# slimgroup/SetIntersectionProjection.jl

Hardware: AMD Instinct MI355X
Metric: PARSDMM iterations/sec (higher is better)
Workload: dtype f32

## Files before the change

setintersectionprojection.jl_amd/csrc/engine.cpp:

```cpp
#include "engine.h"
#include "comm.h"
#include "device_memory.h"
#include "dist_dft.h"
#include "ext_proj.h"
#include "host_prefault.h"
#include "set_config.h"
#include "solve_rules.h"
#include "sparse_granules.h"

#include <algorithm>
#include <array>
#include <chrono>
#include <cmath>
#include <cstdio>
#include <cstdlib>
#include <cstring>
#include <limits>
#include <thread>
#include <exception>

namespace sipx {

const LaunchObserver*& launch_observer() {
  static thread_local const LaunchObserver* obs = nullptr;
// ... 3043 lines not shown
    std::vector<KAgg> agg = aggregate_samples();
    const KAgg& a = stencil_q_ ? agg[KID_SQ_DOT] : agg[KID_CDS_DOT];
    if (launches) *launches = a.launches;
    if (total_ms) *total_ms = a.ms;
    start_stats(enable);
  }
  const char* kernel_stats_json(int enable) override {
    const bool peek = enable < 0;
    if (!peek) need_final();
    std::vector<KAgg> agg = peek ? std::vector<KAgg>(KID_COUNT) : aggregate_samples();
    std::string& o = stats_json_;
    o = "{\"mode\": " + std::to_string(stats_mode_) + ", \"event_pair_overhead_ms\": " + std::to_string(stat_pair_ms_) + ", \"kernels\": [";
    bool first = true;
    char buf[512];
    for (int k = 0; k < KID_COUNT; ++k) {
      if (!agg[k].launches) continue;
      const bool gated = gated_kernel(k);
      std::snprintf(buf, sizeof buf,
                    "%s{\"name\": \"%s\", \"launches\": %lld, \"noop_launches\": %lld, \"total_ms\": %.6f, \"bytes_survey\": %.0f, "
                    "\"bytes_moved\": %.0f, \"gated\": %s, \"inclusive\": %s}",
                    first ? "" : ", ", kernel_name(k), (long long)agg[k].launches, (long long)agg[k].noops, agg[k].ms, agg[k].bytes_survey,
                    agg[k].bytes_moved,
                    gated ? "true" : "false", k == KID_EXT ? "true" : "false");
      o += buf;
      first = false;
    }
    o += "], \"slab_searches\": {\"speculative_exchange\": " + std::to_string(spec_searches_) + ", \"fallbacks\": " +
         std::to_string(spec_fallbacks_) + ", \"refinement_rounds\": " + std::to_string(spec_rounds_) + "}";
    o += std::string(", \"sparse_arrays\": ") + (slab_local_ ? "true" : "false");
    {
      std::string loc, fan;
      for (int i = 0; i < p_n_; ++i) {
        if (sets_[i].slab_ext || sets_[i].slab_card || sets_[i].slab_dft) loc += (loc.empty() ? "" : ", ") + std::to_string(i);
        if (sets_[i].fan) fan += (fan.empty() ? "" : ", ") + std::to_string(i);
      }
      if (counting_)
        o += ", \"collectives\": {\"allreduce\": " + std::to_string(counting_->n_allreduce) + ", \"allreduce_with_halo\": " + std::to_string(counting_->n_grouped) +
             ", \"allgather\": " + std::to_string(counting_->n_allgather) + ", \"reduce_scatter\": " + std::to_string(counting_->n_reduce_scatter) +
             ", \"halo\": " + std::to_string(counting_->n_halo) + ", \"scatter_gather\": " + std::to_string(counting_->n_fan) +
             ", \"alltoall\": " + std::to_string(counting_->n_alltoall) + "}";
      o += ", \"slab_loose\": {\"slab_local_sets\": [" + loc + "], \"gathered_sets\": [" + fan + "], \"fan_exchanges\": " + std::to_string(fan_exchanges_) + "}";
    }
    {
      std::string t = selftest_;
      for (auto& ch : t) if (ch == '"' || ch == '\\' || (unsigned char)ch < 32) ch = ' ';
      o += ", \"comm_selftest\": \"" + t + "\"";
    }
    o += ", \"lane_set\": " + std::to_string(lane_set_);
    o += std::string(", \"q_table\": {\"on\": ") + (cds_.qtab ? "true" : "false") + ", \"reason\": \"" + qtab_reason_ + "\"}";
    o += ", \"batched_searches\": {\"searches\": " + std::to_string(batch_searches_) + ", \"fallbacks\": " + std::to_string(batch_fallbacks_) + "}";
    o += ", \"routes\": {";
    for (int r = 0; r < RT_COUNT; ++r) o += std::string(r ? ", \"" : "\"") + route_name(r) + "\": " + std::to_string(routes_[r]);
    o += "}";
    long long rc[4] = {project_rc_[0], project_rc_[1], project_rc_[2], project_rc_[3]};
    for (const auto& st : sets_) {
      if (!st.ext || st.ext_kind != EXT_RANK) continue;
      long long c[4];
      st.ext->route_counts(c);
      for (int q = 0; q < 4; ++q) rc[q] += c[q];
    }
    o += ", \"rank_route\": {\"calls\": " + std::to_string(rc[0]) + ", \"warm_started_subspace\": " + std::to_string(rc[1]) +
         ", \"full_decomposition\": " + std::to_string(rc[2]) + ", \"products_with_gram\": " + std::to_string(rc[3]) + "}";
    long long fc[4] = {0, 0, 0, 0};
    for (const auto& st : sets_) {
      if (!st.ext || st.ext_kind != EXT_L21_SEG) continue;
      long long c[4];
      st.ext->route_counts(c);
      fc[0] += c[0]; fc[1] = std::max(fc[1], c[1]); fc[3] += c[3];
    }
    o += ", \"l21_frames\": {\"passes_total\": " + std::to_string(fc[0]) + ", \"passes_max\": " + std::to_string(fc[1]) +
         ", \"frames\": " + std::to_string(fc[3]) + "}";
    long long wc[4] = {0, 0, 0, 0};
    for (const auto& st : sets_) {
      if (!st.ext || !st.weighted) continue;
      long long c[4];
      st.ext->route_counts(c);
      for (int q = 0; q < 4; ++q) wc[q] += c[q];
    }
    o += ", \"l21_weighted\": {\"passes\": " + std::to_string(wc[0]) + ", \"flag_reads\": " + std::to_string(wc[1]) +
         ", \"calls\": " + std::to_string(wc[2]) + ", \"groups\": " + std::to_string(wc[3]) + "}}";
    if (!peek) start_stats(enable);
    return o.c_str();
  }
  double stat_pair_overhead_ms() const { return stat_pair_ms_; }

  void debug_proj(int set, int which, double* o) override {
    need_final();
    for (int k = 0; k < 16; ++k) o[k] = 0;
    if (set < 0 || set >= p_n_) throw std::runtime_error("set index out of range");
    const ProjScalars<T>* d = (which & 1) ? sets_[set].psf : sets_[set].ps;
    if (!d) return;
    ProjScalars<T> h;
    SIPX_HIP(hipStreamSynchronize(stream_));
    SIPX_HIP(hipMemcpy(&h, d, sizeof(h), hipMemcpyDeviceToHost));
    o[0] = h.need; o[1] = h.theta; o[2] = h.theta_prev; o[3] = h.hw; o[4] = h.spec_lo; o[5] = h.spec_hi; o[6] = h.lo;
    o[7] = h.hi; o[8] = h.asum; o[9] = h.vmax; o[10] = h.dbg[0]; o[11] = h.dbg[1]; o[12] = h.dbg[2]; o[13] = h.dbg[3];
    o[14] = h.refine;
    o[15] = h.lean + 2 * h.dbg_sampled;
    if (which & 2) { o[4] = h.samp_theta; o[5] = h.samp_lo; o[6] = h.samp_hi; o[7] = h.samp_c; }
  }

  void* stream() override { return (void*)stream_; }
  void* dev_rhs() override { return rhs_; }
  void* dev_x() override { return x_; }
  void get_rhs(void* out) override {
    need_final();
    if (slab_local_ && comm_->world > 1) throw std::runtime_error("a slab-decomposed context holds its planes of rhs only");
    SIPX_HIP(hipStreamSynchronize(stream_));
    SIPX_HIP(hipMemcpy(out, rhs_, Nx_ * sizeof(T), hipMemcpyDeviceToHost));
  }

 private:
  struct KSample { int kid; double bytes_survey, bytes_moved; };
  struct KAgg { long long launches = 0, noops = 0; double ms = 0, bytes_survey = 0, bytes_moved = 0; };
  hipEvent_t stat_event(size_t i) {
    while (stat_ev_.size() <= i) {
      hipEvent_t e;
      SIPX_HIP(hipEventCreate(&e));
      stat_ev_.push_back(e);
    }
    return stat_ev_[i];
  }
  static void obs_begin(void* user, int kid, hipStream_t s, double bytes_survey, double bytes_moved) {
    auto* e = static_cast<Engine<T>*>(user);
    if (e->stats_mode_ == 0 || (e->stats_mode_ == 1 && kid != KID_CDS_DOT && kid != KID_SQ_DOT)) return;
    const size_t i = e->samples_.size();
    e->samples_.push_back(KSample{kid, bytes_survey, bytes_moved});
    e->open_.push_back(i);
    SIPX_HIP(hipEventRecord(e->stat_event(2 * i), s));
  }
  static void obs_end(void* user, int kid, hipStream_t s) {
    auto* e = static_cast<Engine<T>*>(user);
    if (e->stats_mode_ == 0 || (e->stats_mode_ == 1 && kid != KID_CDS_DOT && kid != KID_SQ_DOT)) return;
    if (e->open_.empty()) return;
    const size_t i = e->open_.back();
    e->open_.pop_back();
    if (i < e->samples_.size()) SIPX_HIP(hipEventRecord(e->stat_event(2 * i + 1), s));
  }
  static void obs_route(void* user, int route) {
    if (route >= 0 && route < RT_COUNT) static_cast<Engine<T>*>(user)->routes_[route] += 1;
  }
  void drop_samples_from(size_t n) {
    if (n < samples_.size()) samples_.resize(n);
    open_.clear();
  }
  void sync_all_streams() {
    SIPX_HIP(hipStreamSynchronize(stream_));
    for (hipStream_t q : pool_) if (q != stream_) SIPX_HIP(hipStreamSynchronize(q));
    if (cstream_) SIPX_HIP(hipStreamSynchronize(cstream_));
  }
  static bool gated_kernel(int k) {
    return k == KID_PASS_FIRST || k == KID_PASS_LEAN || k == KID_PASS_PROBE || k == KID_PASS_COMPACT || k == KID_SAMPLE ||
           k == KID_DECIDE || k == KID_CDS_FUSED || k == KID_CG_XR || k == KID_CG_P || k == KID_SLOT_SUMS;
  }
  std::vector<KAgg> aggregate_samples() {
    sync_all_streams();
    std::vector<KAgg> agg(KID_COUNT);
    for (size_t i = 0; i < samples_.size(); ++i) {
      float ms = 0;
      if (hipEventElapsedTime(&ms, stat_ev_[2 * i], stat_ev_[2 * i + 1]) != hipSuccess) { (void)hipGetLastError(); continue; }
      KAgg& a = agg[samples_[i].kid];
      const double t = (double)ms - stat_pair_ms_;
      a.launches += 1;
      a.ms += t > 0 ? t : 0;
      const bool noop = gated_kernel(samples_[i].kid) && samples_[i].bytes_moved > 0 && t * 1e-3 < samples_[i].bytes_moved / 16e12;
      a.noops += noop ? 1 : 0;
      a.bytes_survey += noop ? 0.0 : samples_[i].bytes_survey;
      a.bytes_moved += noop ? 0.0 : samples_[i].bytes_moved;
    }
    return agg;
  }
  void start_stats(int mode) {
    samples_.clear();
    open_.clear();
    stats_mode_ = 0;
    if (mode) {
      std::vector<float> gap;
      for (int k = 0; k < 16; ++k) {
        SIPX_HIP(hipEventRecord(stat_event(2 * k), stream_));
        SIPX_HIP(hipEventRecord(stat_event(2 * k + 1), stream_));
      }
      SIPX_HIP(hipStreamSynchronize(stream_));
      for (int k = 0; k < 16; ++k) {
        float ms = 0;
        SIPX_HIP(hipEventElapsedTime(&ms, stat_ev_[2 * k], stat_ev_[2 * k + 1]));
        gap.push_back(ms);
      }
      std::sort(gap.begin(), gap.end());
      stat_pair_ms_ = gap[gap.size() / 2];
    }
    stats_mode_ = mode;
  }
  const LaunchObserver* observer() const { return &obs_; }
// ... 506 lines not shown
  std::vector<SetState<T>> sets_;
  std::vector<int32_t> owned_;
  bool finalized_ = false, feasibility_only_ = false, any_ncvx_ = false;
  int p_n_ = 0, pp_n_ = 0;
  std::vector<T> rho_, gamma_;
  std::vector<double> feas_init_;
  T *p_base_ = nullptr, *m_base_ = nullptr, *r_base_ = nullptr, *p2_base_ = nullptr, *p2_ = nullptr;
  bool cg_fused_ = false;
  int n_mfree_ = 0;
  long long halo_ = 0;
  T *x_ = nullptr, *xold_ = nullptr, *rhs_ = nullptr, *m_ = nullptr, *r_ = nullptr, *p_ = nullptr, *Ap_ = nullptr;
  T *Q_ = nullptr, *scr_v_ = nullptr, *scr_c_ = nullptr, *maxpart_ = nullptr;
  long long* scr_i_ = nullptr;
  long long scr_c_len_ = 0;
  T* scr_w_ = nullptr;
  T *loose_v_ = nullptr, *loose_w_ = nullptr;
  bool loose_whole_ = false;
  bool need_idx_ = false, need_ext_ = false;
  CdsArgs cds_;
  bool set_streams_ = true;
  hipEvent_t ev_fork_ = nullptr, ev_fork2_ = nullptr;
  std::vector<hipStream_t> pool_;
  bool search_streams_ = false;
  int search_next_ = 0;
  int n_set_streams_ = 2, pool_next_ = 0;
  bool mk_ = false;
  long long Nx_ = 0;
  T *w_base_ = nullptr, *w_ = nullptr;
  StencilQ<T> sq_{};
  bool stencil_q_ = false;
  double *part_cg_ = nullptr, *part_tmp_ = nullptr, *part_sets_ = nullptr;
  CgState<T>*cg_dev_ = nullptr, *cg_host_ = nullptr;
  double* hres_ = nullptr;
  volatile unsigned long long* sums_word_ = nullptr;
  unsigned* sums_ticket_ = nullptr;
  unsigned long long sums_seq_ = 0;
  volatile int* hlean_ = nullptr;
  volatile int* hovf_ = nullptr;
  volatile unsigned* hverd_ = nullptr;
  unsigned spec_seq_ = 0;
  long long spec_searches_ = 0, spec_fallbacks_ = 0, spec_rounds_ = 0;
  int lane_set_ = -1;
  hipStream_t lane_st_ = nullptr;
  hipEvent_t lane_fork_ = nullptr, lane_ev_ = nullptr;
  T* lane_v_ = nullptr;
  std::thread lane_thr_;
  std::exception_ptr lane_err_;
  long long lane_sample_ = -1;
  SetArgs<T> lane_args_;
  bool sweep_partial_ = false, has_loose_ = false;
  bool sweep_plain_ = false;
  bool search_batch_ = false;
  long long batch_searches_ = 0, batch_fallbacks_ = 0;
  long long routes_[RT_COUNT] = {};
  long long project_rc_[4] = {0, 0, 0, 0};
  T* fbuf_ = nullptr;
  bool yl_multi_ = true;
  bool x0_mode_ = false;
  T *xr_base_[3] = {nullptr, nullptr, nullptr}, *xr_[3] = {nullptr, nullptr, nullptr};
  int x_cur_ = 0, x_snap_ = -1;
  bool rhs_fused_ = false;
  hipEvent_t sums_event_ = nullptr;
  std::unique_ptr<Comm> comm_;
  CountingComm* counting_ = nullptr;
  long long plane_ = 0, chunk_ = 0, r0_ = 0, r1_ = 0, qr0_ = 0, qr1_ = 0;
  int prev_ = -1, next_ = -1;
  hipStream_t cstream_ = nullptr;
  hipEvent_t ev_c_[2] = {nullptr, nullptr};
  bool rs_pending_ = false;
  double* dres_ = nullptr;
  hipEvent_t ev_sums_ = nullptr, ev_cgb_ = nullptr;
  bool sums_pending_ = false;
  T* qtab_ = nullptr;
  bool q_stale_ = false;
  std::string qtab_reason_ = "not built";
  DeviceMemory mem_;
  bool slab_dist_logs_ = false;
  bool lean_multi_ = false;
  bool head_done_ = false;
  int merged_nslots_ = 0;
  int sums_flags_ = 0;
  volatile unsigned long long* ticket_ = nullptr;
  unsigned cg_seq_ = 0;
  bool slab_req_ = false, slab_ = false;
  hipStream_t fan_st_ = nullptr;
  hipEvent_t fan_fork_ = nullptr;
  double* fan_ptmp_ = nullptr;
  T *fan_mpart_ = nullptr, *fan_c_ = nullptr;
  long long fan_exchanges_ = 0;
  bool slab_loose_ = false;
  bool slab_full_req_ = false, slab_local_ = false;
  std::string selftest_ = "none", mapped_why_;
  double* agree_buf_ = nullptr;
  bool selftest_mapped_failed_ = false, selftest_alltoall_failed_ = false;
  std::string a2a_why_;
  long long wlo_ = 0, whi_ = 0;
  Grid Gr_, Gyl_;
  ChainHooks hooks_;
  T* gbuf_ = nullptr;
  double *stage_ = nullptr, *sstage_ = nullptr;
  const ChainHooks* hooks() const { return slab_ ? &hooks_ : nullptr; }
  double obj_ss_ = 0, evo_ss_ = 0, xx_ss_ = 0;
  bool have_log_sums_ = false;
  hipEvent_t cg_ev_[2] = {nullptr, nullptr};
  std::vector<hipEvent_t> stat_ev_;
  std::vector<KSample> samples_;
  std::vector<size_t> open_;
// ... 115 lines not shown
```

setintersectionprojection.jl_amd/csrc/kernels_cds.hip:

```cpp
#include <cstdlib>
#include <stdexcept>
#include <string>

#include "sipx_device.h"
#define SIPX_CG_GRID launch_blocks(3)
#ifndef SIPX_F64_VEC
#define SIPX_F64_VEC 2
#endif

namespace sipx {

template <typename T, int V>
struct LoadStored {
  const T* __restrict__ x;
  __device__ __forceinline__ Vec<T, V> operator()(long long c) const { return ldv_u<T, V>(x + c); }
};
template <typename T, int V>
struct LoadFused {
  const T* __restrict__ r;
  const T* __restrict__ p;
  T beta;
  __device__ __forceinline__ Vec<T, V> operator()(long long c) const {
    const Vec<T, V> rv = ldv_u<T, V>(r + c), pv = ldv_u<T, V>(p + c);
    Vec<T, V> o;
#pragma unroll
    for (int k = 0; k < V; ++k) o.v[k] = rv.v[k] + beta * pv.v[k];
    return o;
  }
};

template <typename T, int V, int D, typename XL>
__device__ __forceinline__ void cds_rows(long long N, const T* __restrict__ R, const CdsArgs& a, const XL& xl, long long r,
                                         T (&acc)[V]) {
  const int d = D ? D : a.d;
#pragma unroll
  for (int k = 0; k < V; ++k) acc[k] = T(0);
  if constexpr (D > 0) {
    Vec<T, V> rv[D], xv[D];
#pragma unroll
    for (int b = 0; b < D; ++b) {
      if (a.sym) {
        rv[b] = a.off[b] >= 0 ? ldv<T, V>(R + (long long)b * N + r)
                              : ldv_u<T, V>(R + (long long)a.partner[b] * N + r + a.off[b]);
      } else {
        rv[b] = ldv_nt<T, V>(R + (long long)b * N + r);
      }
      xv[b] = xl(r + a.off[b]);
    }
#pragma unroll
    for (int b = 0; b < D; ++b) {
      const long long c = r + a.off[b];
#pragma unroll
      for (int k = 0; k < V; ++k) {
        const T t = acc[k] + rv[b].v[k] * xv[b].v[k];
        acc[k] = (c + k >= 0 && c + k < N) ? t : acc[k];
      }
// ... 260 lines not shown
        for (int k = 0; k < V; ++k) {
          const T rv[7] = {r0.v[k], k == 0 ? rl : r1.v[k - 1], r1.v[k], ru.v[k], r2.v[k], rzm.v[k], r3.v[k]};
          const T xv[7] = {x0.v[k], k == 0 ? xl : x0.v[k - 1], k == V - 1 ? xr : x0.v[k + 1], xu.v[k], xd.v[k], xm.v[k], xp.v[k]};
          const bool in[7] = {true, k > 0 || !first, k < V - 1 || !last, up, down, below, above};
          T acc = T(0);
#pragma unroll
          for (int q = 0; q < 7; ++q) {
            const int role = march_role(ORD, q);
            const T t = acc + rv[role] * xv[role];
            acc = in[role] ? t : acc;
          }
          o4.v[k] = acc;
        }
        if (MODE == 0) {
          stv_nt<T, V>(y + r, o4);
        } else if (MODE == 1 || MODE == 3) {
#pragma unroll
          for (int k = 0; k < V; ++k) acc0 += (double)x0.v[k] * (double)o4.v[k];
          stv_nt<T, V>(y + r, o4);
          if (MODE == 3) stv<T, V>(pout + r, x0);
        } else {
          Vec<T, V> o;
#pragma unroll
          for (int k = 0; k < V; ++k) {
            o.v[k] = bv.v[k] - o4.v[k];
            acc0 += (double)o.v[k] * (double)o.v[k];
            acc1 += (double)bv.v[k] * (double)bv.v[k];
          }
          stv<T, V>(y + r, o);
          if (pout) stv<T, V>(pout + r, o);
          if (xold) stv<T, V>(xold + r, x0);
        }
      }
      xm = x0; x0 = xp; rzm = r3;
    }
  }
  if (MODE != 0) {
    __shared__ double sm[2][MARCH_NT / 64];
    const double v0 = wave_sum(acc0), v1 = wave_sum(acc1);
    __syncthreads();
    if ((tid & 63) == 0) { sm[0][tid >> 6] = v0; sm[1][tid >> 6] = v1; }
    __syncthreads();
    if (tid < (MODE == 2 ? 2 : 1)) {
      double s = 0;
#pragma unroll
      for (int i = 0; i < MARCH_NT / 64; ++i) s += sm[tid][i];
      double* row = partials + (long long)tid * NB;
      row[blockIdx.x] = s;
      for (int jj = blockIdx.x + gridDim.x; jj < NB; jj += gridDim.x) row[jj] = 0.0;
    }
  }
}

struct MarchGeom {
  int lg, tiles_x, tiles_y, zchunk, grid;
  long long items;
};
template <typename T>
static bool march_geom(long long N, long long r0, long long r1, const CdsArgs& a, MarchGeom& m) {
  const int sw = env_knobs().cds_march;
  const long long zc_env = env_knobs().cds_march_zchunk;
  if (sw == 0 || !a.march || !a.sym || a.d != 7) return false;
  constexpr int V = sizeof(T) == 8 ? 2 : 4;
  const long long n1 = a.gn[0], n2 = a.gn[1], n3 = a.gn[2], st2 = n1 * n2;
  if (n1 % V != 0 || n1 * n2 * n3 != N || r0 % st2 != 0 || r1 % st2 != 0 || r1 <= r0) return false;
  const long long nvx = n1 / V;
  int lg = 0;
  while ((1 << lg) < nvx && lg < 6) ++lg;
  const int LX = 1 << lg, TY = MARCH_NT / LX;
  const int tiles_x = (int)((nvx + LX - 1) / LX), tiles_y = (int)((n2 + TY - 1) / TY);
  const long long tiles = (long long)tiles_x * tiles_y, planes = (r1 - r0) / st2;
  long long zchunk = planes * tiles / 2048;
  if (zchunk < 16) zchunk = 16;
  if (sw == 2 && zc_env > 0) zchunk = zc_env;
  if (zchunk > planes) zchunk = planes;
  const long long nchunks = (planes + zchunk - 1) / zchunk, items = tiles * nchunks;
  if (items < 384 && sw != 2) return false;
  m = MarchGeom{lg, tiles_x, tiles_y, (int)zchunk, (int)(items < NB ? items : NB), items};
  return true;
}
template <typename T>
bool K<T>::march_applies(long long N, const CdsArgs& a) {
  MarchGeom m;
  return march_geom<T>(N, 0, N, a, m);
}

template <typename T, int MODE>
static bool try_march(hipStream_t s, long long N, long long r0, long long r1, const T* R, const CdsArgs& a, const T* x, T* y, const T* b,
                      T* pout, T* xold, double* partials, const int* done, CgState<T>* st = nullptr, CgState<T>* host = nullptr,
                      unsigned long long* ticket = nullptr) {
  MarchGeom m;
  if (!march_geom<T>(N, r0, r1, a, m)) return false;
  constexpr int V = sizeof(T) == 8 ? 2 : 4;
  const long long n1 = a.gn[0], n2 = a.gn[1], n3 = a.gn[2], st2 = n1 * n2;
  const T *R0 = R + (long long)a.mb[0] * N, *R1 = R + (long long)a.mb[1] * N, *R2 = R + (long long)a.mb[2] * N, *R3 = R + (long long)a.mb[3] * N;
#define SIPX_MARCH(ORD, XT, XV)                                                                                                      \
  hipLaunchKernelGGL((k_cds_march<T, V, ORD, MODE, XT>), dim3(m.grid), dim3(MARCH_NT), 0, s, n1, n2, n3, r0 / st2, r1 / st2, R0, R1, R2, R3, x, y, b, \
                     pout, xold, partials, done, m.lg, m.tiles_x, m.tiles_y, m.zchunk, m.items, st, host, ticket, XV)
  if (a.qtab) {
    const QTab<T> tab{(const T*)a.qtab};
    if (a.march == 1) SIPX_MARCH(1, QTab<T>, tab);
    else SIPX_MARCH(2, QTab<T>, tab);
  } else if (a.march == 1) {
    SIPX_MARCH(1, NoExtra, NoExtra{});
  } else {
    SIPX_MARCH(2, NoExtra, NoExtra{});
  }
#undef SIPX_MARCH
  return true;
}

template <typename T, int MODE>
static void launch_cds(hipStream_t s, long long N, long long r0, long long r1, const T* R, const CdsArgs& a, const T* x, T* y,
                       const T* b, T* pout, T* xold, double* partials, const int* done) {
  if (a.d < 1 || a.d > MAXD) throw std::runtime_error("cds: band count out of range");
  if (r0 < 0 || r1 > N || r0 > r1) throw std::runtime_error("cds: row range outside the matrix");
  int read_bands = a.d;
  if (a.sym) { read_bands = 0; for (int b = 0; b < a.d; ++b) read_bands += a.off[b] >= 0 ? 1 : 0; }
  if (a.qtab) read_bands = 0;
  const double rw = (double)(r1 - r0) * sizeof(T), extra = MODE == 2 ? 4.0 : 2.0;
  const double moved_extra = (MODE == 2 && !xold) ? 3.0 : extra;
  ObsScope obs(MODE == 0 ? KID_CDS_SPMV : (MODE == 1 ? KID_CDS_DOT : KID_CDS_RESID), s, (a.d + extra) * rw, (read_bands + moved_extra) * rw);
  if (try_march<T, MODE>(s, N, r0, r1, R, a, x, y, b, pout, xold, partials, done)) {
    obs.route((a.qtab ? RT_CDS_MARCH_TABLE : RT_CDS_MARCH_BANDS) + MODE);
    SIPX_HIP(hipGetLastError());
    return;
  }
  if (a.qtab) throw std::runtime_error("internal: Q's class table is in use but the z-marching product does not apply");
  obs.route(RT_CDS_FLAT + MODE);
#define SIPX_CDS(V, D) \
  hipLaunchKernelGGL((k_cds<T, V, D, MODE>), dim3(fit_grid((r1 - r0) / V, SIPX_CG_GRID)), dim3(BLOCK), 0, s, N, r0, r1, R, a, x, y, b, pout, xold, partials, done)
  constexpr int VW = sizeof(T) == 8 ? SIPX_F64_VEC : 4;
  if (N % 4 == 0 && r0 % 4 == 0 && r1 % 4 == 0) {
    switch (a.d) {
      case 1: SIPX_CDS(VW, 1); break;
      case 3: SIPX_CDS(VW, 3); break;
      case 5: SIPX_CDS(VW, 5); break;
      case 7: SIPX_CDS(VW, 7); break;
      default: SIPX_CDS(VW, 0); break;
    }
  } else {
    SIPX_CDS(1, 0);
  }
#undef SIPX_CDS
  SIPX_HIP(hipGetLastError());
}

template <typename T>
void K<T>::spmv(hipStream_t s, const Grid&, long long N, const T* R, const CdsArgs& a, const T* x, T* y) {
  launch_cds<T, 0>(s, N, 0, N, R, a, x, y, nullptr, nullptr, nullptr, nullptr, nullptr);
}
template <typename T>
void K<T>::spmv_dot(hipStream_t s, long long N, long long r0, long long r1, const T* R, const CdsArgs& a, const T* p, T* Ap,
                    double* partials, const CgState<T>* st) {
  launch_cds<T, 1>(s, N, r0, r1, R, a, p, Ap, nullptr, nullptr, nullptr, partials, &st->done);
}
template <typename T>
void K<T>::resid(hipStream_t s, long long N, long long r0, long long r1, const T* R, const CdsArgs& a, const T* x, const T* b,
                 T* r, T* p, T* xold, double* partials) {
  launch_cds<T, 2>(s, N, r0, r1, R, a, x, r, b, p, xold, partials, nullptr);
}

template <typename T, int V>
__device__ __forceinline__ void stencil_rows(const Grid& G, const StencilQ<T>& q, const T* __restrict__ x, long long g,
                                             const Vec<T, V>& xc, T (&acc)[V]) {
  const Coord c = coords(G, g);
#pragma unroll
  for (int k = 0; k < V; ++k) acc[k] = q.w0 * xc.v[k];
#pragma unroll
  for (int dir = 0; dir < 3; ++dir) {
    if (!(q.mask & (1 << dir))) continue;
    const long long st = G.st[dir];
    const int nd = (int)G.n[dir], cd = coord_of(c, dir);
    const Vec<T, V> xm = ldv_u<T, V>(x + g - st), xp = ldv_u<T, V>(x + g + st);
#pragma unroll
    for (int k = 0; k < V; ++k) {
      const int ck = cd + (dir == 0 ? k : 0);
// ... 623 lines not shown
template <typename T, int V, int D>
__global__ __launch_bounds__(BLOCK) void k_cds_fused(long long N, const T* __restrict__ R, CdsArgs a, const T* __restrict__ r,
                                                     const T* __restrict__ p_old, T* __restrict__ p_new, T* __restrict__ Ap,
                                                     double* __restrict__ partials, CgState<T>* __restrict__ st,
                                                     CgState<T>* __restrict__ host, unsigned long long* ticket) {
  if (st->done) return;
  const double ss = block_sum_partials(partials + NB);
  const T rr = (T)ss;
  const T res = (T)sqrt(ss) / st->nr0;
  const bool conv = res <= st->tol;
  const T beta = rr / st->gamma;
  if (blockIdx.x == 0 && threadIdx.x == 0) {
    st->ss = ss;
    st->res_last = res;
    if (conv) {
      st->flag = 0;
      st->done = 1;
    } else {
      st->beta = beta;
    }
    st->rr = rr;
    *host = *st;
    publish_ticket(ticket, st->seq, st->iters, conv ? 1 : 0);
  }
  if (conv) return;
  const LoadFused<T, V> xl{r, p_old, beta};
  const long long nvec = N / V;
  double acc0 = 0;
  for (long long vi = (long long)blockIdx.x * BLOCK + threadIdx.x; vi < nvec; vi += (long long)gridDim.x * BLOCK) {
    const long long row = vi * V;
    T s[V];
    cds_rows<T, V, D>(N, R, a, xl, row, s);
    const Vec<T, V> pv = xl(row);
    Vec<T, V> o;
#pragma unroll
    for (int k = 0; k < V; ++k) {
      o.v[k] = s[k];
      acc0 += (double)pv.v[k] * (double)s[k];
    }
    stv<T, V>(p_new + row, pv);
    stv_nt<T, V>(Ap + row, o);
  }
  double acc[1] = {acc0};
  block_reduce_store<1>(acc, partials, 0);
}
template <typename T>
void K<T>::spmv_fused(hipStream_t s, long long N, const T* R, const CdsArgs& a, const T* r, const T* p_old, T* p_new, T* Ap,
                      double* partials, CgState<T>* st, CgState<T>* host, unsigned long long* ticket) {
  if (a.d < 1 || a.d > MAXD) throw std::runtime_error("cds: band count out of range");
  int read_bands = a.d;
  if (a.sym) { read_bands = 0; for (int b = 0; b < a.d; ++b) read_bands += a.off[b] >= 0 ? 1 : 0; }
  if (a.qtab) read_bands = 0;
  ObsScope obs(KID_CDS_FUSED, s, (a.d + 4.0) * (double)N * sizeof(T), (read_bands + 4.0) * (double)N * sizeof(T));
  if (try_march<T, 3>(s, N, 0, N, R, a, r, Ap, p_old, p_new, nullptr, partials, nullptr, st, host, ticket)) {
    obs.route((a.qtab ? RT_CDS_MARCH_TABLE : RT_CDS_MARCH_BANDS) + 3);
    SIPX_HIP(hipGetLastError());
    return;
  }
  if (a.qtab) throw std::runtime_error("internal: Q's class table is in use but the z-marching product does not apply");
  obs.route(RT_CDS_FUSED_FLAT);
#define SIPX_CDSF(V, D) \
  hipLaunchKernelGGL((k_cds_fused<T, V, D>), dim3(fit_grid(N / V, SIPX_CG_GRID)), dim3(BLOCK), 0, s, N, R, a, r, p_old, p_new, Ap, partials, st, host, ticket)
  constexpr int VW = sizeof(T) == 8 ? SIPX_F64_VEC : 4;
  if (N % 4 == 0) {
    switch (a.d) {
      case 1: SIPX_CDSF(VW, 1); break;
      case 3: SIPX_CDSF(VW, 3); break;
      case 5: SIPX_CDSF(VW, 5); break;
      case 7: SIPX_CDSF(VW, 7); break;
      default: SIPX_CDSF(VW, 0); break;
    }
  } else {
    SIPX_CDSF(1, 0);
  }
#undef SIPX_CDSF
  SIPX_HIP(hipGetLastError());
}

__global__ __launch_bounds__(BLOCK) void k_fin_sum(const double* __restrict__ partials, double* __restrict__ out_dev,
                                                   double* __restrict__ out_host, unsigned* __restrict__ ticket,
                                                   unsigned long long* __restrict__ word, unsigned long long seq) {
  const double s = block_sum_partials(partials + (long long)blockIdx.x * NB);
  if (threadIdx.x == 0) {
    if (out_dev) out_dev[blockIdx.x] = s;
    if (out_host) out_host[blockIdx.x] = s;
    if (word) {
      __threadfence_system();
      const unsigned t = __hip_atomic_fetch_add(ticket, 1u, __ATOMIC_ACQ_REL, __HIP_MEMORY_SCOPE_AGENT);
      if (t == gridDim.x - 1) {
        __hip_atomic_store(ticket, 0u, __ATOMIC_RELAXED, __HIP_MEMORY_SCOPE_AGENT);
        __threadfence_system();
        __hip_atomic_store(word, seq, __ATOMIC_RELEASE, __HIP_MEMORY_SCOPE_SYSTEM);
      }
    }
  }
}
template <typename T>
void K<T>::fin_sum(hipStream_t s, const double* partials, int nslots, double* out_dev, double* out_host, unsigned* ticket,
                   unsigned long long* word, unsigned long long seq) {
  ObsScope obs(KID_FIN_SUM, s, (double)nslots * NB * sizeof(double));
  hipLaunchKernelGGL(k_fin_sum, dim3(nslots), dim3(BLOCK), 0, s, partials, out_dev, out_host, ticket, word, seq);
  SIPX_HIP(hipGetLastError());
}

__global__ __launch_bounds__(BLOCK) void k_copy_f64(const double* __restrict__ src, double* __restrict__ dst, int n) {
  for (int i = threadIdx.x; i < n; i += BLOCK) dst[i] = src[i];
}
template <typename T>
// ... 38 lines not shown
```

setintersectionprojection.jl_amd/csrc/sipx_common.h:

```cpp
#pragma once
#include <hip/hip_runtime.h>
#include <stdint.h>
#include <cstdio>

#include "env_knobs.h"

namespace sipx {

constexpr int BLOCK = 256;
constexpr int NB = 2048;
constexpr int NB_7 = 1792;
inline int fit_grid(long long nvec, int cap) {
  const long long need = (nvec + BLOCK - 1) / BLOCK;
  return (int)(need < 1 ? 1 : (need < cap ? need : cap));
}
template <typename... P>
inline bool aligned16(const P*... p) {
  return (((reinterpret_cast<uintptr_t>(p) & 15u) == 0) && ...);
}
inline int launch_blocks(int per_cu) {
  static const int cus = [] {
    int dev = 0, n = 0;
    if (hipGetDevice(&dev) != hipSuccess || hipDeviceGetAttribute(&n, hipDeviceAttributeMultiprocessorCount, dev) != hipSuccess || n <= 0)
      n = 256;
    return n;
  }();
  const int g = per_cu * cus;
  return g < 256 ? 256 : (g > NB_7 ? NB_7 : g);
}
constexpr int MAXD = 32;
constexpr int MAX_SETS = 16;
constexpr int QT_N = 4 * 27;
constexpr int YL_SLOTS = 13;
constexpr int L1_K = 8;
#define SIPX_SOLVE_SLOTS 64
#define SIPX_MAX_WORLD 64
constexpr int GATHER_HDR = 8;
constexpr int PREP_SLOTS = 3 + 2 * L1_K;
template <typename T>
constexpr int fast_hdr() { return ((PREP_SLOTS + 4) * 8 / (int)sizeof(T) + 3) / 4 * 4; }
constexpr int SAMPLE_BINS = 1024;
constexpr int SAMPLE_MBITS = 7;

enum KernelId {
  KID_CDS_SPMV = 0, KID_CDS_DOT, KID_CDS_RESID, KID_CDS_FUSED, KID_SQ_SPMV, KID_SQ_DOT, KID_SQ_RESID, KID_CG_BEGIN, KID_CG_XR, KID_CG_P,
  KID_Q_UPDATE, KID_FIN_SUM, KID_RHS, KID_YL, KID_YL_MULTI, KID_ADJ_NORM, KID_LOG3, KID_PASS_FIRST, KID_PASS_LEAN, KID_PASS_PROBE,
  KID_PASS_COMPACT, KID_PASS_DIST, KID_PASS_STORE, KID_PASS_MULTI, KID_SLOT_SUMS, KID_DECIDE, KID_SAMPLE, KID_L1_SOLVE, KID_GATHER,
  KID_PS_RESCALE, KID_CARD, KID_EXT, KID_BB_RULE, KID_OTHER, KID_MF_FWD, KID_MF_ADJ, KID_L21_NORMS, KID_L21_FRAMES, KID_L21_SCALE,
  KID_L21J_NORMS, KID_L21J_FINISH, KID_L21J_SCALE, KID_L21W_PASS, KID_L21W_SCALE, KID_COUNT
};
inline const char* kernel_name(int k) {
  static const char* const names[KID_COUNT] = {
      "k_cds<MODE=0>", "k_cds<MODE=1>", "k_cds<MODE=2>", "k_cds_fused", "k_sq<MODE=0>", "k_sq<MODE=1>", "k_sq<MODE=2>", "k_cg_begin",
      "k_cg_update_xr", "k_cg_update_p", "k_q_update", "k_fin_sum", "k_rhs", "k_yl", "k_yl_multi", "k_adj_norm", "k_log3",
      "k_pass<M_FIRST>", "k_pass<M_LEAN>", "k_pass<M_PROBE>", "k_pass<M_COMPACT>", "k_pass<M_DIST>", "k_pass<M_STORE>", "k_pass_multi",
      "k_slot_sums", "k_decide", "k_sample", "k_l1_solve", "k_gather_pack/unpack", "k_ps_rescale", "k_card_*", "ext_proj (library-backed)",
      "k_bb_rule", "other", "k_mf_fwd", "k_mf_adj", "k_l21_norms", "k_l21_frames", "k_l21_scale",
      "k_l21j_norms", "k_l21j_finish", "k_l21j_scale", "k_l21w_part", "k_l21w_scale"};
  return (k >= 0 && k < KID_COUNT) ? names[k] : "?";
}
enum RouteId {
  RT_CDS_MARCH_BANDS = 0,
  RT_CDS_MARCH_TABLE = 4,
  RT_CDS_FLAT = 8,
  RT_CDS_FUSED_FLAT = 11,
  RT_RHS_MARCH = 12,
  RT_RHS_FLAT = 13,
  RT_COUNT = 14
};
inline const char* route_name(int r) {
  static const char* const names[RT_COUNT] = {
      "k_cds_march<MODE=0>/bands", "k_cds_march<MODE=1>/bands", "k_cds_march<MODE=2>/bands", "k_cds_march<MODE=3>/bands",
      "k_cds_march<MODE=0>/table", "k_cds_march<MODE=1>/table", "k_cds_march<MODE=2>/table", "k_cds_march<MODE=3>/table",
      "k_cds<MODE=0>", "k_cds<MODE=1>", "k_cds<MODE=2>", "k_cds_fused", "k_rhs_march", "k_rhs"};
  return (r >= 0 && r < RT_COUNT) ? names[r] : "?";
}
struct LaunchObserver {
  void* user;
  void (*begin)(void* user, int kid, hipStream_t s, double bytes_survey, double bytes_moved);
  void (*end)(void* user, int kid, hipStream_t s);
  void (*route)(void* user, int route);
};
const LaunchObserver*& launch_observer();

struct ObsScope {
  const LaunchObserver* o;
  int kid;
  hipStream_t s;
  ObsScope(int kid_, hipStream_t s_, double bytes_survey, double bytes_moved = -1.0) : o(launch_observer()), kid(kid_), s(s_) {
    if (env_knobs().trace_kernels) fprintf(stderr, "[sipx trace] %s\n", kernel_name(kid));
    if (o) o->begin(o->user, kid, s, bytes_survey, bytes_moved < 0 ? bytes_survey : bytes_moved);
  }
  ~ObsScope() {
    if (o) o->end(o->user, kid, s);
    if (env_knobs().trace_kernels) {
      (void)hipStreamSynchronize(s);
      fprintf(stderr, "[sipx trace]   done\n");
    }
  }
  void route(int r) const { if (o && o->route) o->route(o->user, r); }
  ObsScope(const ObsScope&) = delete;
  ObsScope& operator=(const ObsScope&) = delete;
};

enum { SL_RPRI = 0, SL_DY = 1, SL_HL = 2, SL_HH = 3, SL_LH = 4, SL_DL = 5, SL_GG = 6, SL_GL = 7,
       SL_FE = 8, SL_SS = 9, SL_OBJ = 10, SL_EVO = 11, SL_XX = 12,
       SL_ADJ = 13 , SL_FE2 = 14, SL_SS2 = 15  };
constexpr int SET_SLOTS = 16;

enum { F_FEAS = 1, F_BB = 2, F_FIRST = 4, F_NOSPEC = 8 ,
       F_STORE_DY = 16  };

enum { PX_BOUNDS = 0, PX_BOUNDS_VEC = 1, PX_L1 = 2, PX_L2 = 3, PX_ANNULUS = 4, PX_CARD = 5, PX_PROX_L1 = 6,
       PX_EXT = 8,
       PX_DIST = 100 };

struct Grid {
  long long n[3];
  long long N;
  long long st[3];
  unsigned m1 = 0, s1 = 0, m2 = 0, s2 = 0;
// ... 433 lines not shown
```

Before: 866.6.

## Add LDS ring-buffered z-marching CDS kernel using async global-to-LDS loads

Adds a variant of the z-marching 7-point stencil SpMV that streams planes into a multi-slot LDS ring buffer with global_load_lds, fetching several planes ahead. Waits use explicit vmcnt counts so loads overlap compute instead of holding neighbour planes in registers. A heuristic picks it for f32 with the class table when there are enough work items, and route counters record which load path ran. It relies on hand-computed outstanding-load counts and inline asm, so miscounted waits could cause races, and the larger LDS footprint limits occupancy to two workgroups per CU.

```diff
diff --git a/setintersectionprojection.jl_amd/csrc/engine.cpp b/setintersectionprojection.jl_amd/csrc/engine.cpp
--- a/setintersectionprojection.jl_amd/csrc/engine.cpp
+++ b/setintersectionprojection.jl_amd/csrc/engine.cpp
@@ -3119,6 +3119,7 @@
     o += ", \"routes\": {";
     for (int r = 0; r < RT_COUNT; ++r) o += std::string(r ? ", \"" : "\"") + route_name(r) + "\": " + std::to_string(routes_[r]);
     o += "}";
+    o += ", \"march_loads\": {\"ring\": " + std::to_string(routes_[RT_LOADS_RING]) + ", \"registers\": " + std::to_string(routes_[RT_LOADS_REGISTERS]) + "}";
     long long rc[4] = {project_rc_[0], project_rc_[1], project_rc_[2], project_rc_[3]};
     for (const auto& st : sets_) {
       if (!st.ext || st.ext_kind != EXT_RANK) continue;
@@ -3205,7 +3206,7 @@
     if (i < e->samples_.size()) SIPX_HIP(hipEventRecord(e->stat_event(2 * i + 1), s));
   }
   static void obs_route(void* user, int route) {
-    if (route >= 0 && route < RT_COUNT) static_cast<Engine<T>*>(user)->routes_[route] += 1;
+    if (route >= 0 && route < RT_ALL) static_cast<Engine<T>*>(user)->routes_[route] += 1;
   }
   void drop_samples_from(size_t n) {
     if (n < samples_.size()) samples_.resize(n);
@@ -3818,7 +3819,7 @@
   bool sweep_plain_ = false;
   bool search_batch_ = false;
   long long batch_searches_ = 0, batch_fallbacks_ = 0;
-  long long routes_[RT_COUNT] = {};
+  long long routes_[RT_ALL] = {};
   long long project_rc_[4] = {0, 0, 0, 0};
   T* fbuf_ = nullptr;
   bool yl_multi_ = true;
diff --git a/setintersectionprojection.jl_amd/csrc/kernels_cds.hip b/setintersectionprojection.jl_amd/csrc/kernels_cds.hip
--- a/setintersectionprojection.jl_amd/csrc/kernels_cds.hip
+++ b/setintersectionprojection.jl_amd/csrc/kernels_cds.hip
@@ -2,6 +2,7 @@
 #include <stdexcept>
 #include <string>
 
+#include "march_ring.h"
 #include "sipx_device.h"
 #define SIPX_CG_GRID launch_blocks(3)
 #ifndef SIPX_F64_VEC
@@ -368,13 +369,294 @@
   }
 }
 
+template <typename T, int MODE, int D>
+struct RingLds {
+  static constexpr int NVEC = MODE == 3 ? 2 : 1;
+  static constexpr int EW = (int)sizeof(T) / 4;
+  static constexpr int MAIN = (MARCH_NT + 2 * 64) * 16;
+  static constexpr int VEC = MAIN + EW * MARCH_NT * 4;
+  static constexpr int SLOT = NVEC * VEC + (MODE == 2 ? MARCH_NT * 16 : 0);
+  static constexpr int CTAB = ring::slots(D) * SLOT;
+  static constexpr int SM = CTAB + (QT_N * (int)sizeof(T) + 15) / 16 * 16;
+  static constexpr int BYTES = SM + 2 * (MARCH_NT / 64) * (int)sizeof(double);
+};
+#define SIPX_GLDS(NAME, BYTES)                                                                                          \
+  __device__ __forceinline__ void NAME(const void* src, unsigned char* wave_base) {                                     \
+    __builtin_amdgcn_global_load_lds((const __attribute__((address_space(1))) void*)src,                                \
+                                     (__attribute__((address_space(3))) void*)wave_base, BYTES, 0, 0);                 \
+  }
+SIPX_GLDS(glds16, 16)
+SIPX_GLDS(glds4, 4)
+#undef SIPX_GLDS
+typedef unsigned ring_u4 __attribute__((ext_vector_type(4)));
+__device__ __forceinline__ unsigned lds_offset(const unsigned char* p) {
+  return (unsigned)(unsigned long long)(const __attribute__((address_space(3))) unsigned char*)p;
+}
+__device__ __forceinline__ ring_u4 lds_ld16(unsigned at) {
+  ring_u4 v;
+  asm volatile("ds_read_b128 %0, %1" : "=v"(v) : "v"(at) : "memory");
+  return v;
+}
+__device__ __forceinline__ unsigned lds_ld4(unsigned at) {
+  unsigned v;
+  asm volatile("ds_read_b32 %0, %1" : "=v"(v) : "v"(at) : "memory");
+  return v;
+}
+__device__ __forceinline__ void lds_landed() { asm volatile("s_waitcnt lgkmcnt(0)" ::: "memory"); }
+__device__ __forceinline__ void pin(ring_u4& v) { asm volatile("" : "+v"(v)::"memory"); }
+__device__ __forceinline__ void pin(unsigned& v) { asm volatile("" : "+v"(v)::"memory"); }
+__device__ __forceinline__ void wait_vm(int n) {
+#define SIPX_VM(N) case N: asm volatile("s_waitcnt vmcnt(" #N ")" ::: "memory"); break;
+  switch (__builtin_amdgcn_readfirstlane(n)) {
+    SIPX_VM(0) SIPX_VM(1) SIPX_VM(2) SIPX_VM(3) SIPX_VM(4) SIPX_VM(5) SIPX_VM(6) SIPX_VM(7) SIPX_VM(8) SIPX_VM(9) SIPX_VM(10) SIPX_VM(11)
+    SIPX_VM(12) SIPX_VM(13) SIPX_VM(14) SIPX_VM(15) SIPX_VM(16) SIPX_VM(17) SIPX_VM(18) SIPX_VM(19) SIPX_VM(20) SIPX_VM(21) SIPX_VM(22)
+    SIPX_VM(23)
+    default: asm volatile("s_waitcnt vmcnt(24)" ::: "memory"); break;
+  }
+#undef SIPX_VM
+}
+template <typename T, int V, int ORD, int MODE, int D>
+__global__ __launch_bounds__(MARCH_NT) void k_cds_march_ring(long long n1, long long n2, long long n3, long long z0, long long z1,
+                                                             const T* __restrict__ x, T* __restrict__ y, const T* __restrict__ b,
+                                                             T* __restrict__ pout, T* __restrict__ xold, double* __restrict__ partials,
+                                                             const int* __restrict__ done, int lgLX, int tiles_x, int tiles_y, int zchunk,
+                                                             long long items, CgState<T>* __restrict__ st, CgState<T>* __restrict__ host,
+                                                             unsigned long long* ticket, QTab<T> extra) {
+  using LY = RingLds<T, MODE, D>;
+  static_assert(sizeof(Vec<T, V>) == 16 && D >= 1 && D <= ring::MAX_D, "16-byte entries, one to three planes ahead");
+  if (MODE == 1 && *done) return;
+  T beta = T(0);
+  if (MODE == 3) {
+    if (st->done) return;
+    const double ss = block_sum_partials_n<MARCH_NT>(partials + NB);
+    const T rr = (T)ss;
+    const T res = (T)sqrt(ss) / st->nr0;
+    const bool conv = res <= st->tol;
+    beta = rr / st->gamma;
+    if (blockIdx.x == 0 && threadIdx.x == 0) {
+      st->ss = ss;
+      st->res_last = res;
+      if (conv) { st->flag = 0; st->done = 1; } else { st->beta = beta; }
+      st->rr = rr;
+      *host = *st;
+      publish_ticket(ticket, st->seq, st->iters, conv ? 1 : 0);
+    }
+    if (conv) return;
+  }
+  __shared__ __attribute__((aligned(16))) unsigned char lds[LY::BYTES];
+  T* ctab = reinterpret_cast<T*>(lds + LY::CTAB);
+  load_class_tab(extra, ctab);
+  __syncthreads();
+  const int tid = threadIdx.x, LX = 1 << lgLX, tx = tid & (LX - 1), ty = tid >> lgLX, TY = MARCH_NT >> lgLX;
+  const int wave = __builtin_amdgcn_readfirstlane(tid >> 6);
+  constexpr int LASTW = MARCH_NT / 64 - 1;
+  const long long st1 = n1, st2 = n1 * n2, N = st2 * n3;
+  const long long tiles = (long long)tiles_x * tiles_y;
+  const bool whole_rows = tiles_x == 1 && n1 == (long long)LX * V;
+  const bool halo_wave = wave == 0 || wave == LASTW;
+  const int hrow = ty == 0 ? -1 : (ty == TY - 1 ? 1 : 0), ecol = tx == 0 ? -1 : (tx == LX - 1 ? V : 0);
+  const int L = LY::NVEC * (1 + (halo_wave ? 1 : 0) + (whole_rows ? 0 : LY::EW)) + (MODE == 2 ? 1 : 0);
+  const int S_all = MODE == 2 ? 1 + (pout ? 1 : 0) + (xold ? 1 : 0) : (MODE == 3 ? 2 : 1);
+  const int own = (LX + tid) * 16;
+  double acc0 = 0, acc1 = 0;
+  for (long long item = blockIdx.x; item < items; item += gridDim.x) {
+    const long long zc = item / tiles, tile = item - zc * tiles;
+    const int tile_y = (int)(tile / tiles_x), tile_x = (int)(tile - (long long)tile_y * tiles_x);
+    const long long i0 = ((long long)tile_x * LX + tx) * V, j = (long long)tile_y * TY + ty;
+    const bool active = i0 < n1 && j < n2;
+    const long long k0 = z0 + zc * zchunk, k1 = (k0 + zchunk < z1) ? k0 + zchunk : z1;
+    const long long go = active ? i0 + st1 * j : 0;
+    const long long go_wrap = (i0 < n1 && j == n2) ? i0 + st1 * j : go;
+    const long long go_halo = active ? go + hrow * st1 : go, go_edge = active ? go + ecol : go;
+    const int S = __ballot(active) != 0 ? S_all : 0;
+    auto fetch = [&](long long p) {
+      unsigned char* sl = lds + ring::slot(p, k0, D) * LY::SLOT;
+      const bool inner = p >= k0 && p < k1;
+      const long long pz = st2 * p;
+#pragma unroll
+      for (int q = 0; q < LY::NVEC; ++q) {
+        const T* src = (q == 0 ? x : b) + pz;
+        unsigned char* vs = sl + q * LY::VEC;
+        glds16(src + (p < k1 ? go_wrap : go), vs + (LX + 64 * wave) * 16);
+        if (halo_wave) {
+          if (hrow != 0) glds16(src + (inner ? go_halo : go), vs + (wave == 0 ? 0 : MARCH_NT + 2 * LX - 64) * 16);
+        }
+        if (!whole_rows) {
+          if (ecol != 0) {
+#pragma unroll
+            for (int w = 0; w < LY::EW; ++w)
+              glds4(reinterpret_cast<const unsigned*>(src + (inner ? go_edge : go)) + w, vs + LY::MAIN + (w * MARCH_NT + 64 * wave) * 4);
+          }
+        }
+      }
+      if (MODE == 2) {
+        const long long pb = p < k0 ? k0 : (p < k1 ? p : k1 - 1);
+        glds16(b + st2 * pb + go, sl + LY::VEC + 64 * wave * 16);
+      }
+    };
+    struct Raw { ring_u4 v[LY::NVEC]; };
+    auto read_at = [&](unsigned sl, int at) -> Raw {
+      Raw w;
+#pragma unroll
+      for (int q = 0; q < LY::NVEC; ++q) w.v[q] = lds_ld16(sl + q * LY::VEC + at);
+      return w;
+    };
+    auto form = [&](Raw& w) -> Vec<T, V> {
+      Vec<T, V> v;
+      pin(w.v[0]);
+      __builtin_memcpy(&v, &w.v[0], 16);
+      if (MODE == 3) {
+        Vec<T, V> pv;
+        pin(w.v[LY::NVEC - 1]);
+        __builtin_memcpy(&pv, &w.v[LY::NVEC - 1], 16);
+#pragma unroll
+        for (int k = 0; k < V; ++k) v.v[k] = v.v[k] + beta * pv.v[k];
+      }
+      return v;
+    };
+    struct RawPoint { unsigned u[LY::NVEC][LY::EW]; };
+    auto read_point = [&](unsigned sl, int at, int step) -> RawPoint {
+      RawPoint w;
+#pragma unroll
+      for (int q = 0; q < LY::NVEC; ++q)
+#pragma unroll
+        for (int k = 0; k < LY::EW; ++k) w.u[q][k] = lds_ld4(sl + q * LY::VEC + at + k * step);
+      return w;
+    };
+    auto form_point = [&](RawPoint& w) -> T {
+      T e[LY::NVEC];
+#pragma unroll
+      for (int q = 0; q < LY::NVEC; ++q) {
+#pragma unroll
+        for (int k = 0; k < LY::EW; ++k) pin(w.u[q][k]);
+        __builtin_memcpy(&e[q], w.u[q], sizeof(T));
+      }
+      return MODE == 3 ? e[0] + beta * e[LY::NVEC - 1] : e[0];
+    };
+    const int at_left = whole_rows ? own - (int)sizeof(T) : LY::MAIN + tid * 4, at_right = whole_rows ? own + 16 : at_left;
+    const int at_step = whole_rows ? 4 : MARCH_NT * 4;
+    const unsigned ring0 = lds_offset(lds);
+    auto slot_at = [&](long long p) -> unsigned { return ring0 + ring::slot(p, k0, D) * LY::SLOT; };
+    asm volatile("s_waitcnt lgkmcnt(0)" ::: "memory");
+    __builtin_amdgcn_s_barrier();
+    for (long long p = k0 - 1; p <= ring::last_before_loop(k0, k1, D); ++p) fetch(p);
+    Vec<T, V> xm = zerov<T, V>(), x0 = zerov<T, V>(), rzm = zerov<T, V>();
+    if (active && k0 > 0) rzm = tab_row<T, V>(ctab, 3, 3 * line_class(j, n2) + 9 * line_class(k0 - 1, n3), i0, n1);
+    for (long long kz = k0; kz < k1; ++kz) {
+      wait_vm(ring::wait_plane(kz, k0, k1, D, L, S));
+      asm volatile("s_waitcnt lgkmcnt(0)" ::: "memory");
+      __builtin_amdgcn_s_barrier();
+      asm volatile("" ::: "memory");
+      if (kz == k0) {
+        Raw wm = read_at(slot_at(k0 - 1), own), w0 = read_at(slot_at(k0), own);
+        lds_landed();
+        const Vec<T, V> vm = form(wm), v0 = form(w0);
+        if (active) { xm = vm; x0 = v0; }
+      }
+      const long long nf = ring::fetch_at(kz, k1, D);
+      if (nf >= 0) fetch(nf);
+      asm volatile("" ::: "memory");
+      const unsigned sl = slot_at(kz), sn = slot_at(kz + 1);
+      const long long pz = st2 * kz;
+      Vec<T, V> xp = zerov<T, V>(), r0 = xp, r1 = xp, r2 = xp, r3 = xp, bv = xp;
+      const int cz = line_class(kz, n3), cyz = 3 * line_class(j, n2) + 9 * cz;
+      const int cyz_up = j > 0 ? 3 * line_class(j - 1, n2) + 9 * cz : 3 * line_class(n2 - 1, n2) + 9 * line_class(kz - 1, n3);
+      Raw wp = read_at(sn, own);
+      RawPoint wl = read_point(sl, at_left, at_step), wr = read_point(sl, at_right, at_step);
+      ring_u4 wb;
+      if (MODE == 2) wb = lds_ld16(sl + LY::VEC + tid * 16);
+      lds_landed();
+      const T el = form_point(wl), er = form_point(wr);
+      if (active) {
+        xp = form(wp);
+        r0 = tab_row<T, V>(ctab, 0, cyz, i0, n1);
+        r1 = tab_row<T, V>(ctab, 1, cyz, i0, n1);
+        r2 = tab_row<T, V>(ctab, 2, cyz, i0, n1);
+        r3 = tab_row<T, V>(ctab, 3, cyz, i0, n1);
+        if (MODE == 2) { pin(wb); __builtin_memcpy(&bv, &wb, 16); }
+      }
+      T xl = __shfl_up(x0.v[V - 1], 1, 64), xr = __shfl_down(x0.v[0], 1, 64), rl = T(0);
+      const long long r = pz + go;
+      if (r > 0) rl = i0 > 0 ? ctab[27 + line_class(i0 - 1, n1) + cyz] : ctab[27 + line_class(n1 - 1, n1) + cyz_up];
+      Raw wu = read_at(sl, own - LX * 16), wd = read_at(sl, own + LX * 16);
+      lds_landed();
+      if (active) {
+        if (tx == 0) xl = el;
+        if (tx == LX - 1) xr = er;
+        Vec<T, V> ru = zerov<T, V>();
+        if (r - st1 >= 0) ru = tab_row<T, V>(ctab, 2, cyz_up, i0, n1);
+        const Vec<T, V> xu = form(wu), xd = form(wd);
+        const bool up = r >= st1, down = r + st1 < N, below = r >= st2, above = r + st2 < N, first = r == 0, last = r + V == N;
+        Vec<T, V> o4;
+#pragma unroll
+        for (int k = 0; k < V; ++k) {
+          const T rv[7] = {r0.v[k], k == 0 ? rl : r1.v[k - 1], r1.v[k], ru.v[k], r2.v[k], rzm.v[k], r3.v[k]};
+          const T xv[7] = {x0.v[k], k == 0 ? xl : x0.v[k - 1], k == V - 1 ? xr : x0.v[k + 1], xu.v[k], xd.v[k], xm.v[k], xp.v[k]};
+          const bool in[7] = {true, k > 0 || !first, k < V - 1 || !last, up, down, below, above};
+          T acc = T(0);
+#pragma unroll
+          for (int q = 0; q < 7; ++q) {
+            const int role = march_role(ORD, q);
+            const T t = acc + rv[role] * xv[role];
+            acc = in[role] ? t : acc;
+          }
+          o4.v[k] = acc;
+        }
+        if (MODE == 0) {
+          stv_nt<T, V>(y + r, o4);
+        } else if (MODE == 1 || MODE == 3) {
+#pragma unroll
+          for (int k = 0; k < V; ++k) acc0 += (double)x0.v[k] * (double)o4.v[k];
+          stv_nt<T, V>(y + r, o4);
+          if (MODE == 3) stv<T, V>(pout + r, x0);
+        } else {
+          Vec<T, V> o;
+#pragma unroll
+          for (int k = 0; k < V; ++k) {
+            o.v[k] = bv.v[k] - o4.v[k];
+            acc0 += (double)o.v[k] * (double)o.v[k];
+            acc1 += (double)bv.v[k] * (double)bv.v[k];
+          }
+          stv<T, V>(y + r, o);
+          if (pout) stv<T, V>(pout + r, o);
+          if (xold) stv<T, V>(xold + r, x0);
+        }
+      }
+      xm = x0; x0 = xp; rzm = r3;
+    }
+  }
+  if (MODE != 0) {
+    double(*sm)[MARCH_NT / 64] = reinterpret_cast<double(*)[MARCH_NT / 64]>(lds + LY::SM);
+    const double v0 = wave_sum(acc0), v1 = wave_sum(acc1);
+    __syncthreads();
+    if ((tid & 63) == 0) { sm[0][tid >> 6] = v0; sm[1][tid >> 6] = v1; }
+    __syncthreads();
+    if (tid < (MODE == 2 ? 2 : 1)) {
+      double s = 0;
+#pragma unroll
+      for (int i = 0; i < MARCH_NT / 64; ++i) s += sm[tid][i];
+      double* row = partials + (long long)tid * NB;
+      row[blockIdx.x] = s;
+      for (int jj = blockIdx.x + gridDim.x; jj < NB; jj += gridDim.x) row[jj] = 0.0;
+    }
+  }
+}
+
+static int march_switch() {
+  const int v = env_knobs().cds_march;
+  return v == 3 ? 1 : (v == 4 || v == 5 ? 2 : v);
+}
+static int ring_switch() {
+  const int v = env_knobs().cds_march;
+  return v == 3 || v == 4 ? 0 : (v == 5 ? 2 : 1);
+}
 struct MarchGeom {
   int lg, tiles_x, tiles_y, zchunk, grid;
   long long items;
 };
 template <typename T>
 static bool march_geom(long long N, long long r0, long long r1, const CdsArgs& a, MarchGeom& m) {
-  const int sw = env_knobs().cds_march;
+  const int sw = march_switch();
   const long long zc_env = env_knobs().cds_march_zchunk;
   if (sw == 0 || !a.march || !a.sym || a.d != 7) return false;
   constexpr int V = sizeof(T) == 8 ? 2 : 4;
@@ -401,15 +683,47 @@
   return march_geom<T>(N, 0, N, a, m);
 }
 
+constexpr int CU_LDS_BYTES = 160 * 1024;
 template <typename T, int MODE>
-static bool try_march(hipStream_t s, long long N, long long r0, long long r1, const T* R, const CdsArgs& a, const T* x, T* y, const T* b,
-                      T* pout, T* xold, double* partials, const int* done, CgState<T>* st = nullptr, CgState<T>* host = nullptr,
-                      unsigned long long* ticket = nullptr) {
+constexpr int march_ring_depth() {
+  if (MODE == 3 && sizeof(T) == 8) return 0;
+  return MODE == 0 || MODE == 1 ? 2 : 1;
+}
+template <typename T, int MODE>
+static bool march_ring_pays(const MarchGeom& m) {
+  const int sw = ring_switch();
+  if (sw == 0 || march_ring_depth<T, MODE>() == 0) return false;
+  if (sw == 2) return true;
+  if (sizeof(T) != 4) return false;
+  return MODE == 3 || (MODE != 2 && m.items > launch_blocks(2));
+}
+template <typename T, int V, int ORD, int MODE, int D>
+static void launch_march_ring(hipStream_t s, const MarchGeom& m, long long n1, long long n2, long long n3, long long z0, long long z1, const T* x,
+                              T* y, const T* b, T* pout, T* xold, double* partials, const int* done, CgState<T>* st, CgState<T>* host,
+                              unsigned long long* ticket, const QTab<T>& tab) {
+  static_assert(2 * RingLds<T, MODE, D>::BYTES <= CU_LDS_BYTES, "two workgroups per CU");
+  hipLaunchKernelGGL((k_cds_march_ring<T, V, ORD, MODE, D>), dim3(m.grid), dim3(MARCH_NT), 0, s, n1, n2, n3, z0, z1, x, y, b, pout, xold, partials,
+                     done, m.lg, m.tiles_x, m.tiles_y, m.zchunk, m.items, st, host, ticket, tab);
+}
+
+template <typename T, int MODE>
+static int try_march(hipStream_t s, long long N, long long r0, long long r1, const T* R, const CdsArgs& a, const T* x, T* y, const T* b,
+                     T* pout, T* xold, double* partials, const int* done, CgState<T>* st = nullptr, CgState<T>* host = nullptr,
+                     unsigned long long* ticket = nullptr) {
   MarchGeom m;
-  if (!march_geom<T>(N, r0, r1, a, m)) return false;
+  if (!march_geom<T>(N, r0, r1, a, m)) return 0;
   constexpr int V = sizeof(T) == 8 ? 2 : 4;
   const long long n1 = a.gn[0], n2 = a.gn[1], n3 = a.gn[2], st2 = n1 * n2;
   const T *R0 = R + (long long)a.mb[0] * N, *R1 = R + (long long)a.mb[1] * N, *R2 = R + (long long)a.mb[2] * N, *R3 = R + (long long)a.mb[3] * N;
+  constexpr int D = march_ring_depth<T, MODE>();
+  if constexpr (D > 0) {
+    if (a.qtab && march_ring_pays<T, MODE>(m)) {
+      const QTab<T> tab{(const T*)a.qtab};
+      if (a.march == 1) launch_march_ring<T, V, 1, MODE, D>(s, m, n1, n2, n3, r0 / st2, r1 / st2, x, y, b, pout, xold, partials, done, st, host, ticket, tab);
+      else launch_march_ring<T, V, 2, MODE, D>(s, m, n1, n2, n3, r0 / st2, r1 / st2, x, y, b, pout, xold, partials, done, st, host, ticket, tab);
+      return 2;
+    }
+  }
 #define SIPX_MARCH(ORD, XT, XV)                                                                                                      \
   hipLaunchKernelGGL((k_cds_march<T, V, ORD, MODE, XT>), dim3(m.grid), dim3(MARCH_NT), 0, s, n1, n2, n3, r0 / st2, r1 / st2, R0, R1, R2, R3, x, y, b, \
                      pout, xold, partials, done, m.lg, m.tiles_x, m.tiles_y, m.zchunk, m.items, st, host, ticket, XV)
@@ -423,7 +737,11 @@
     SIPX_MARCH(2, NoExtra, NoExtra{});
   }
 #undef SIPX_MARCH
-  return true;
+  return 1;
+}
+static void book_march(const ObsScope& obs, const CdsArgs& a, int mode, int how) {
+  obs.route((a.qtab ? RT_CDS_MARCH_TABLE : RT_CDS_MARCH_BANDS) + mode);
+  if (a.qtab) obs.route(how == 2 ? RT_LOADS_RING : RT_LOADS_REGISTERS);
 }
 
 template <typename T, int MODE>
@@ -437,8 +755,8 @@
   const double rw = (double)(r1 - r0) * sizeof(T), extra = MODE == 2 ? 4.0 : 2.0;
   const double moved_extra = (MODE == 2 && !xold) ? 3.0 : extra;
   ObsScope obs(MODE == 0 ? KID_CDS_SPMV : (MODE == 1 ? KID_CDS_DOT : KID_CDS_RESID), s, (a.d + extra) * rw, (read_bands + moved_extra) * rw);
-  if (try_march<T, MODE>(s, N, r0, r1, R, a, x, y, b, pout, xold, partials, done)) {
-    obs.route((a.qtab ? RT_CDS_MARCH_TABLE : RT_CDS_MARCH_BANDS) + MODE);
+  if (const int how = try_march<T, MODE>(s, N, r0, r1, R, a, x, y, b, pout, xold, partials, done)) {
+    book_march(obs, a, MODE, how);
     SIPX_HIP(hipGetLastError());
     return;
   }
@@ -1168,8 +1486,8 @@
   if (a.sym) { read_bands = 0; for (int b = 0; b < a.d; ++b) read_bands += a.off[b] >= 0 ? 1 : 0; }
   if (a.qtab) read_bands = 0;
   ObsScope obs(KID_CDS_FUSED, s, (a.d + 4.0) * (double)N * sizeof(T), (read_bands + 4.0) * (double)N * sizeof(T));
-  if (try_march<T, 3>(s, N, 0, N, R, a, r, Ap, p_old, p_new, nullptr, partials, nullptr, st, host, ticket)) {
-    obs.route((a.qtab ? RT_CDS_MARCH_TABLE : RT_CDS_MARCH_BANDS) + 3);
+  if (const int how = try_march<T, 3>(s, N, 0, N, R, a, r, Ap, p_old, p_new, nullptr, partials, nullptr, st, host, ticket)) {
+    book_march(obs, a, 3, how);
     SIPX_HIP(hipGetLastError());
     return;
   }
diff --git a/setintersectionprojection.jl_amd/csrc/march_ring.h b/setintersectionprojection.jl_amd/csrc/march_ring.h
--- /dev/null
+++ b/setintersectionprojection.jl_amd/csrc/march_ring.h
@@ -0,0 +1,27 @@
+#pragma once
+
+#ifdef __HIPCC__
+#define SIPX_RING_HD __host__ __device__
+#else
+#define SIPX_RING_HD
+#endif
+
+namespace sipx {
+namespace ring {
+
+constexpr int MAX_D = 3;
+SIPX_RING_HD constexpr int slots(int D) { return D + 2; }
+SIPX_RING_HD constexpr int slot(long long plane, long long k0, int D) { return (int)((plane - (k0 - 1)) % (D + 2)); }
+SIPX_RING_HD constexpr long long last_before_loop(long long k0, long long k1, int D) { return k0 + D < k1 ? k0 + D : k1; }
+SIPX_RING_HD constexpr long long last_plane(long long , long long k1) { return k1; }
+SIPX_RING_HD constexpr long long fetch_at(long long kz, long long k1, int D) { return kz + 1 + D <= k1 ? kz + 1 + D : -1; }
+SIPX_RING_HD constexpr int outstanding(long long q, long long fetched, long long kz, long long k0, int D, int L, int S) {
+  const long long from = q - 1 - D > k0 ? q - 1 - D : k0;
+  return (int)((fetched - q) * L + (kz - from) * S);
+}
+SIPX_RING_HD constexpr int wait_plane(long long kz, long long k0, long long k1, int D, int L, int S) {
+  return outstanding(kz + 1, kz + D < k1 ? kz + D : k1, kz, k0, D, L, S);
+}
+
+}
+}
diff --git a/setintersectionprojection.jl_amd/csrc/sipx_common.h b/setintersectionprojection.jl_amd/csrc/sipx_common.h
--- a/setintersectionprojection.jl_amd/csrc/sipx_common.h
+++ b/setintersectionprojection.jl_amd/csrc/sipx_common.h
@@ -66,7 +66,10 @@
   RT_CDS_FUSED_FLAT = 11,
   RT_RHS_MARCH = 12,
   RT_RHS_FLAT = 13,
-  RT_COUNT = 14
+  RT_COUNT = 14,
+  RT_LOADS_RING = 14,
+  RT_LOADS_REGISTERS = 15,
+  RT_ALL = 16
 };
 inline const char* route_name(int r) {
   static const char* const names[RT_COUNT] = {
```

After: 866.7 (median of 5 runs). No clear change (+0.0%).
